# VITA-Group/MM3DGS-SLAM

Hardware: AMD Instinct MI355X
Metric: SLAM frames/sec (track+map), TUM fr1/desk-shaped 640x480 (higher is better)
Workload: dtype f32

## Files before the change

### mm3dgs_slam_amd/csrc/api.hip

```cpp
#include <math.h>
#include <stdarg.h>
#include <stdio.h>
#include <string.h>
#include "mm3dgs_common.h"
#include <algorithm>
#include "fused_api.h"

static thread_local char g_err[512] = "";
static int fail(int code, const char* fmt, ...) {
  va_list ap;
  va_start(ap, fmt);
  vsnprintf(g_err, sizeof(g_err), fmt, ap);
  va_end(ap);
  return code;
}
static int check_launch(const char* what) {
  hipError_t e = hipGetLastError();
  if (e != hipSuccess) return fail(-10, "%s: %s", what, hipGetErrorString(e));
  return 0;
}

#include <mutex>
#include <vector>
struct KernelProfile {
// ... 233 lines not shown
         P > 0 && d.slot_bits >= DIRECT_SLOT_BITS_MIN && T <= max_tiles && T <= MAX_LDS_TILES && d.bin_cap >= 32 && d.rec_cap >= 1024 && d.trec_cap >= 256 &&
         N_capacity >= 4 * (size_t)P;
  return d;
}

static bool slam_tile_table(int flags) { return (flags & MM3DGS_FWD_STATE_CLEAN) && !env_flag("MM3DGS_NO_TILE_ORDER", 0); }
static void slam_refresh_tile_order(const Mm3dgsCamera* cam, void* image_state, int flags, void* stream) {
  if (!cam || !image_state || !slam_tile_table(flags) || cam->image_height <= 0 || cam->image_width <= 0) return;
  if (flags & MM3DGS_FWD_KEEP_TILE_ORDER) return;
  const CamDev cd = cam_dev(cam);
  launch_tile_order(cd.gx * cd.gy, cd.H, cd.W, image_view(image_state, cd.H, cd.W), (hipStream_t)stream);
}

static int slam_forward_impl(const Mm3dgsCamera* cam, int P, const Mm3dgsSlamInputs* in, float* out_color, int32_t* radii,
                             void* geom_state, void* image_state, void* binning_state, size_t N_capacity, int flags, void* stream,
                             const TrackLoss* tl, float* track_dsub = nullptr, bool projected = false, bool pose_chain = false) {
  int rc = check_slam(cam, P, in);
  if (rc) return rc;
  if (!out_color || !geom_state || !image_state || !binning_state || (P > 0 && !radii)) return fail(-1, "NULL buffer");
  hipStream_t s = (hipStream_t)stream;
  CamDev cd = cam_dev(cam);
  GeomView g = geom_view(geom_state, P > 0 ? P : 1);
  ImageView iv = image_view(image_state, cd.H, cd.W);
  BinView b = bin_view(binning_state, N_capacity);
  if (!(flags & MM3DGS_FWD_STATE_CLEAN))
    if (hipMemsetAsync(image_state, 0, iv.zero_bytes, s) != hipSuccess) return fail(-10, "memset failed");
  cd.sort_single = (flags & MM3DGS_FWD_SHORT_LISTS) ? 1 : 0;
  cd.bg_extras = 1;
  cd.state_clean = (flags & MM3DGS_FWD_STATE_CLEAN) ? 1 : 0;
  cd.tile_table = slam_tile_table(flags) ? 1 : 0;
  cd.fused_scan = ((flags & MM3DGS_FWD_STATE_CLEAN) && P > 0 && cd.gx * cd.gy <= MAX_FUSED_SCAN_TILES && !env_flag("MM3DGS_NO_FUSED_SCAN", 0)) ? 1 : 0;
  const bool fused_sort = slam_fused_sort(flags);
  if (tl && !fused_sort) return fail(-1, "internal: folded tracking loss needs the fused sort path");
  const DirectBins db = slam_direct_bins(flags, cd, P, N_capacity);
  cd.trec_cap = db.on ? db.trec_cap : 0u;
  if (db.on) {
    if (!projected) { ProfScope ps(MM3DGS_PROF_PREPROCESS_FWD, s); launch_slam_project_bin(cd, P, slam_in(in), radii, g, iv, b, db.bin_cap, db.rec_cap, db.slot_bits, s, pose_chain); }
    { ProfScope ps(track_dsub ? MM3DGS_PROF_TRACK_FWD_BWD : MM3DGS_PROF_COMPOSITE_FWD, s);
      if (track_dsub) launch_sort_composite_fwd_bwd_track(cd, g, iv, b, N_capacity, out_color, 1, s, *tl, db.nblocks, track_dsub, db.bin_cap, db.slot_bits, pose_chain);
      else launch_sort_composite_fwd6(cd, g, iv, b, N_capacity, out_color, 1, s, tl, db.nblocks, db.bin_cap, db.slot_bits); }
    return check_launch("slam_forward");
  }
  { ProfScope ps(MM3DGS_PROF_PREPROCESS_FWD, s); launch_slam_preprocess_fwd(cd, P, slam_in(in), radii, g, iv, s, nullptr, false, pose_chain); }
  if (!cd.fused_scan) { ProfScope ps(MM3DGS_PROF_SCAN, s); launch_scan_tiles(cd.gx * cd.gy, P, g, iv, s, (flags & MM3DGS_FWD_STATE_CLEAN) ? 1 : 0); }
  { ProfScope ps(MM3DGS_PROF_BIN_SORT, s); launch_scatter_sort(cd, P, g, iv, b, N_capacity, nullptr, s, fused_sort); }
  { ProfScope ps((fused_sort && track_dsub) ? MM3DGS_PROF_TRACK_FWD_BWD : MM3DGS_PROF_COMPOSITE_FWD, s);
    if (fused_sort && track_dsub) launch_sort_composite_fwd_bwd_track(cd, g, iv, b, N_capacity, out_color, (cd.fused_scan || cd.state_clean) ? 1 : 0, s, *tl, 0, track_dsub, 0, DIRECT_SLOT_BITS_MAX, pose_chain);
    else if (fused_sort) launch_sort_composite_fwd6(cd, g, iv, b, N_capacity, out_color, (cd.fused_scan || cd.state_clean) ? 1 : 0, s, tl);
    else launch_composite_fwd(cd, 6, g, iv, b, N_capacity, out_color, s); }
  return check_launch("slam_forward");
}

int mm3dgs_slam_visibility(const Mm3dgsCamera* cam, int P, const Mm3dgsSlamInputs* in, int32_t* radii, uint32_t* seen_count, void* geom_state,
                           void* stream) {
  int rc = check_slam(cam, P, in);
  if (rc) return rc;
  if (!geom_state || (P > 0 && !radii)) return fail(-1, "NULL buffer");
  CamDev cd = cam_dev(cam);
  GeomView g = geom_view(geom_state, P > 0 ? P : 1);
  ImageView iv = {};
  launch_slam_preprocess_fwd(cd, P, slam_in(in), radii, g, iv, (hipStream_t)stream, seen_count, true);
  return check_launch("slam_visibility");
// ... 156 lines not shown
    tl.gt = gt_color; tl.ref = ref; tl.out = out_color; tl.sums = (const double*)w;
    tl.partial = (double*)(w + 256 + align_up((size_t)9 * loss_cfg->H * loss_cfg->W * 4, 256));
    tl.loss4 = loss4;
    tl.defer_scale = loss_cfg->w_pearson == 0.f ? 1 : 0;
    if (loss_cfg->H != cam->image_height || loss_cfg->W != cam->image_width) return fail(-1, "loss and camera image sizes differ");
  }
  const bool fuse_track = fold && tl.defer_scale && !env_flag("MM3DGS_NO_FUSED_TRACK", 0) && backward_scratch;
  float* track_dsub = nullptr;
  if (fuse_track) {
    track_dsub = bwd_view(backward_scratch, P, N_capacity).dsub;
  }
  const bool pose_chain = !in->world_means && !sh && backward_scratch && !env_flag("MM3DGS_NO_POSE_CHAIN", 0) &&
                          bwd_bytes_impl(P, N_capacity) >= (size_t)tiles_x(cam->image_width) * tiles_y(cam->image_height) * 32 * sizeof(float);
  if (n_iter > 0) slam_refresh_tile_order(cam, image_state, fwd_flags, stream);
  for (int it = 0; it < n_iter; it++) {
    int rc = slam_forward_impl(cam, P, in, out_color, radii, geom_state, image_state, binning_state, N_capacity, fwd_flags, stream, fold ? &tl : nullptr, track_dsub, false, pose_chain);
    if (rc) return rc;
    if (fold) {
      if (!tl.defer_scale) {
        ProfScope ps(MM3DGS_PROF_LOSS, (hipStream_t)stream);
        launch_loss_finish(tl.cfg, (double*)loss_work, tl.partial, (hipStream_t)stream);
      }
    } else {
      rc = mm3dgs_loss(loss_cfg, out_color, gt_color, ref, loss_work, dL_dout, loss4, stream);
      if (rc) return rc;
    }
    rc = slam_backward_impl(cam, P, in, radii, geom_state, image_state, binning_state, N_capacity, dL_dout, backward_scratch, &none,
                            nullptr, pose_adam, nullptr, fwd_flags, stream, fold ? &tl : nullptr, loss4, 6, fuse_track, nullptr, nullptr, pose_chain);
    if (rc) return rc;
  }
  return 0;
// ... 229 lines not shown
```

### mm3dgs_slam_amd/csrc/composite.hip

```cpp
#include <type_traits>
#include "mm3dgs_common.h"
#include "sort_tile.h"
#include "fused_api.h"
#include "loss_pixel.h"
#include "loss_tile.h"

#define STG_ROW 17
#define STG_N (4 * STG_ROW)

#include "composite_common.h"

template <int C>
__device__ __forceinline__ void composite_fwd_body(int tile, const CamDev& cam, const GeomView& g, const ImageView& iv, const BinView& b,
                                                   uint32_t N_cap, float* __restrict__ out, float4 (*stg)[4][3][STG_N],
                                                   const uint32_t* counts_lds, const TrackLoss* tl = nullptr,
                                                   double (*red)[12] = nullptr, const SortShared* span = nullptr) {
  const int tid = threadIdx.x, lane = tid & 63, wv = tid >> 6;
  const int row = lane >> 4, q = lane & 15;
  const int slane = row * STG_ROW + q;
  const int px = (tile % cam.gx) * TILE + (wv & 1) * 8 + (row & 1) * 4 + (q & 3);
  const int py = (tile / cam.gx) * TILE + (wv >> 1) * 8 + (row >> 1) * 4 + (q >> 2);
  const bool inside = px < cam.W && py < cam.H;
  const float pxf = (float)px, pyf = (float)py;
  uint32_t start, len;
  if (span) { start = span->start; len = span->len; }
  else tile_span(iv, tile, N_cap, start, len);
  const int L = 4 * wv + row;
  const uint32_t count = len ? min(counts_lds ? counts_lds[L] : iv.subcount[NLIST * tile + L], len) : 0u;
  uint32_t maxcount = count;
  maxcount = max(maxcount, (uint32_t)__builtin_amdgcn_readlane((int)count, 16));
  maxcount = max(maxcount, (uint32_t)__builtin_amdgcn_readlane((int)count, 32));
// ... 62 lines not shown
        splat_fwd(A1, B1, C1, j1);
      }
    }
    if (__ballot(!done && base + CH < count) == 0ull) break;
    stg[cur ^ 1][wv][0][slane] = rec_n.A;
    stg[cur ^ 1][wv][1][slane] = rec_n.B;
    if (C > 2) stg[cur ^ 1][wv][2][slane] = rec_n.C;
    id_nxt = id_nn;
  }
  wave_prio_reset();
  if (cam.stats && lane == 0) atomicAdd(&iv.hdr->fwd_wave_iters, n_iter);
  float fin[C];
#pragma unroll
  for (int ch = 0; ch < C; ch++) fin[ch] = acc[ch] + ((ch < 3 || cam.bg_extras) ? Tr * cam.bg[ch % 3] : 0.f);
  const size_t pix = (size_t)py * cam.W + px, HW = (size_t)cam.H * cam.W;
  if (inside) {
    iv.final_T[pix] = Tr;
    iv.n_contrib[pix] = last_contributor;
#pragma unroll
    for (int ch = 0; ch < C; ch++) out[ch * HW + pix] = fin[ch];
  }
  if constexpr (C == 6) {
    if (tl) {
      double ls[12];
#pragma unroll
      for (int k = 0; k < 12; k++) ls[k] = 0.0;
      if (inside) {
        const float rgb[3] = {fin[0], fin[1], fin[2]};
        const float g3[3] = {tl->gt[pix], tl->gt[HW + pix], tl->gt[2 * HW + pix]};
        loss_px_sums(tl->cfg, rgb, fin[4], fin[3], g3, tl->cfg.w_pearson != 0.f ? tl->ref[pix] : 0.f, ls);
      }
      block_sums<12>(ls, red, pearson_double_cols(tl->cfg));
      if (threadIdx.x == 0) {
        double* rowp = tl->partial + (size_t)tile * 12;
#pragma unroll
        for (int k = 0; k < 12; k++) rowp[k] = ls[k];
      }
    }
  }
}

template <int C>
__global__ void __launch_bounds__(256)
composite_fwd_kernel(CamDev cam, GeomView g, ImageView iv, BinView b, uint32_t N_cap, float* __restrict__ out) {
  __shared__ float4 stg[2][4][3][STG_N];
// ... 92 lines not shown
  static constexpr int OFF_CZ = OFF_B + STG_N * 16;
  static constexpr int OFF_TP = OFF_CZ + STG_N * 8;
  static constexpr int OFF_T5 = OFF_TP + 4 * TP_STRIDE * 8;
  static constexpr int OFF_T = OFF_TP + 8 * TP_STRIDE * 8;
  static constexpr int SLICE = OFF_T + (MODE == 1 ? 64 * 16 : 64 * 4);
};
template <int MODE>
using BwdLds = Bwd2Lds<(MODE == 0 ? 1 : MODE)>;
template <int C, int MODE>
constexpr size_t BWD_WAVE_SLICE = bwd_is_two_phase(MODE, C) ? (size_t)BwdLds<MODE>::SLICE : sizeof(float4) * 3 * STG_N;
template <int C, int MODE>
constexpr size_t BWD_LDS_BYTES = bwd_is_two_phase(MODE, C) ? 4 * (size_t)BwdLds<MODE>::SLICE : (size_t)BWD_STG_BYTES;
template <int C, int MODE, bool POSE = false>
__device__ __forceinline__ void composite_bwd_body(int tile, const CamDev& cam, const GeomView& g, const ImageView& iv, const BinView& b,
                                                   uint32_t N_cap, const float* __restrict__ dL_dout, float* __restrict__ dsub, int has_tl,
                                                   const TrackLoss& tl, int dl_planes, unsigned char* smem_raw, const SortShared* span = nullptr) {
  static_assert(!POSE || MODE == 2, "the pose chain lives in the tracking mode's loop");
  const int tid = threadIdx.x, lane = tid & 63, wv = tid >> 6;
  const int row = lane >> 4, q = lane & 15;
  const int slane = row * STG_ROW + q;
  const int px = (tile % cam.gx) * TILE + (wv & 1) * 8 + (row & 1) * 4 + (q & 3);
  const int py = (tile / cam.gx) * TILE + (wv >> 1) * 8 + (row >> 1) * 4 + (q >> 2);
  const bool inside = px < cam.W && py < cam.H;
  const float pxf = (float)px, pyf = (float)py;
  uint32_t start, len;
  if (span) { start = span->start; len = span->len; }
  else tile_span(iv, tile, N_cap, start, len);
  const int L = 4 * wv + row;
  const uint32_t count = len ? min(span ? span->run[L] : iv.subcount[NLIST * tile + L], len) : 0u;
  const uint2* __restrict__ list = b.sublist + (size_t)NLIST * start + (size_t)L * len;

  constexpr int NV = MODE == 0 ? 6 + C : (MODE == 1 ? 10 : 7);
  static_assert(MODE == 0 || C == 6, "SLAM modes composite the 6-channel bundle");
  constexpr int RECF = MODE == 0 ? GENERIC_RECF(C) : (MODE == 1 ? REC_MAP_F : REC_TRACK_F);
  float4 (*stg)[4][3][STG_N] = (float4 (*)[4][3][STG_N])smem_raw;
  constexpr uint32_t CH = 16;

  const size_t pix = (size_t)py * cam.W + px, HW = (size_t)cam.H * cam.W;
  const float T_final = inside ? iv.final_T[pix] : 0.f;
  const uint32_t last_contributor = inside ? iv.n_contrib[pix] : 0u;
  uint32_t todo = last_contributor;
  todo = max(todo, (uint32_t)__builtin_amdgcn_update_dpp(0, (int)todo, QP_XOR1, 0xf, 0xf, true));
  todo = max(todo, (uint32_t)__builtin_amdgcn_update_dpp(0, (int)todo, QP_XOR2, 0xf, 0xf, true));
  todo = max(todo, (uint32_t)__builtin_amdgcn_update_dpp(0, (int)todo, ROW_ROR4, 0xf, 0xf, true));
  todo = max(todo, (uint32_t)__builtin_amdgcn_update_dpp(0, (int)todo, ROW_ROR8, 0xf, 0xf, true));
  todo = min(todo, count);
  const uint32_t maxtodo = max(max((uint32_t)__builtin_amdgcn_readlane((int)todo, 0), (uint32_t)__builtin_amdgcn_readlane((int)todo, 16)),
                               max((uint32_t)__builtin_amdgcn_readlane((int)todo, 32), (uint32_t)__builtin_amdgcn_readlane((int)todo, 48)));
  float dL[C];
  float bg_dot = 0.f;
  bool dl_done = false;
  if constexpr (MODE == 2) {
    if (has_tl) {
#pragma unroll
      for (int ch = 0; ch < C; ch++) dL[ch] = 0.f;
      if (inside) {
        const float sil = tl.out[4 * HW + pix];
        const bool smask = sil > tl.cfg.sil_thr;
        const float l1s = tl.defer_scale ? tl.cfg.w_l1 / 3.f : loss_l1_scale(tl.cfg, tl.sums);
#pragma unroll
        for (int ch = 0; ch < 3; ch++) dL[ch] = loss_px_l1_grad(tl.cfg, tl.out[ch * HW + pix], tl.gt[ch * HW + pix], smask, l1s);
        if (tl.cfg.w_pearson != 0.f) dL[3] = loss_px_pearson_grad(tl.cfg, sil, tl.out[3 * HW + pix], tl.ref[pix], tl.sums);
      }
      if (!tl.defer_scale && tile == 0 && threadIdx.x == 0 && tl.loss4) loss_scalars(tl.cfg, tl.sums, HW, tl.loss4);
      dl_done = true;
    }
  }
  if constexpr (MODE == 1) {
    if (has_tl) {
      LossGradSmem& lsm = *(LossGradSmem*)smem_raw;
      float* exch = (float*)(smem_raw + sizeof(LossGradSmem));
      float g4[4];
      bool in_raster;
      if (PROBE(cam, 10)) { g4[0] = g4[1] = g4[2] = g4[3] = 1e-3f; in_raster = true; }
      else loss_grad_tile(tl.cfg, tl.out, tl.gt, tl.ref, tl.dmaps, tl.sums, tile, cam.gx, lsm, g4, in_raster);
#pragma unroll
      for (int ch = 0; ch < 4; ch++) exch[ch * 256 + tid] = g4[ch];
// ... 492 lines not shown
  constexpr size_t LOSS_BYTES = MODE == 1 ? sizeof(LossGradSmem) + 4 * 256 * sizeof(float) : 0;
  constexpr size_t MIN_BYTES = MODE == 0 ? 32768 : 0;
  constexpr size_t STG_BYTES = BWD_LDS_BYTES<C, MODE>;
  constexpr size_t NEED = STG_BYTES > LOSS_BYTES ? STG_BYTES : LOSS_BYTES;
  __shared__ __align__(16) unsigned char smem_raw[NEED > MIN_BYTES ? NEED : MIN_BYTES];
  const int T = cam.gx * cam.gy;
  const int tile = slam_tile(cam, iv, blockIdx.x, T);
  if (tile >= T) return;
  if (MODE == 1 && blockIdx.x == 0 && threadIdx.x == 0) iv.hdr->overflow_seen = iv.hdr->overflow;
  composite_bwd_body<C, MODE, POSE>(tile, cam, g, iv, b, N_cap, dL_dout, dsub, has_tl, tl, dl_planes, smem_raw);
}

template <bool POSE>
__global__ void __launch_bounds__(256) __attribute__((amdgpu_waves_per_eu(5, 5)))
sort_composite_fwd_bwd_track_kernel(CamDev cam, GeomView g, ImageView iv, BinView b, uint32_t N_cap, float* __restrict__ out, int clean,
                                    TrackLoss tl, int direct_blocks, float* __restrict__ dsub, uint32_t direct_cap, int slot_bits) {
  constexpr size_t TRACK_BWD_BYTES = BWD_LDS_BYTES<6, 2>;
  __shared__ __align__(16) unsigned char smem[TRACK_BWD_BYTES];
  __shared__ SortShared sh;
  __shared__ double red[4][12];
  static_assert(TRACK_BWD_BYTES >= sizeof(float4) * 2 * 4 * 3 * STG_N, "LDS union too small for the forward staging buffers");
  static_assert(TRACK_BWD_BYTES >= 3 * RANK_SORT_MAX * sizeof(unsigned long long) + sizeof(SortEmit), "LDS union too small for the sort's keys, runs, payloads and the emission's counters");
  const int T = cam.gx * cam.gy;
  const int tile = slam_tile(cam, iv, blockIdx.x, T);
  if (tile >= T) return;
  sort_tile_body<2048, true>(tile, cam.gx, 0, g, iv, b, N_cap, clean, (unsigned long long*)smem, sh, 0, direct_blocks, direct_cap, slot_bits);
  __syncthreads();
  composite_fwd_body<6>(tile, cam, g, iv, b, N_cap, out, (float4 (*)[4][3][STG_N])smem, sh.run, &tl, red, &sh);
  __syncthreads();
  composite_bwd_body<6, 2, POSE>(tile, cam, g, iv, b, N_cap, nullptr, dsub, 1, tl, 6, smem, &sh);
}

template <int C>
static void launch_fwd_c(const CamDev& cam, GeomView g, ImageView iv, BinView b, uint32_t ncap, float* out, hipStream_t s) {
  int T = cam.gx * cam.gy;
  int grid = ((T + 7) / 8) * 8;
  static const int pad = env_flag("MM3DGS_FWD_LDS_PAD", 0);
  hipLaunchKernelGGL((composite_fwd_kernel<C>), dim3(grid), dim3(256), (size_t)pad, s, cam, g, iv, b, ncap, out);
}
template <int C>
static void launch_bwd_c(const CamDev& cam, GeomView g, ImageView iv, BinView b, uint32_t ncap, const float* dL, float* dsub,
                         hipStream_t s) {
  int T = cam.gx * cam.gy;
  int grid = ((T + 7) / 8) * 8;
  TrackLoss none = {};
// ... 13 lines not shown
    hipLaunchKernelGGL((composite_bwd_kernel<6, 2>), dim3(grid), dim3(256), slam_lds_pad(), s, cam, g, iv, b, ncap, dL, dsub, tl ? 1 : 0, tl ? *tl : none, dl_planes);
  else
    hipLaunchKernelGGL((composite_bwd_kernel<6, 1>), dim3(grid), dim3(256), slam_lds_pad(), s, cam, g, iv, b, ncap, dL, dsub, tl ? 1 : 0, tl ? *tl : none, dl_planes);
}

void launch_sort_composite_fwd6(const CamDev& cam, GeomView g, ImageView iv, BinView b, size_t N_cap, float* out, int clean, hipStream_t s,
                                const TrackLoss* tl, int direct_blocks, uint32_t direct_cap, int slot_bits) {
  uint32_t ncap = (uint32_t)(N_cap > 0xffffffffull ? 0xffffffffull : N_cap);
  int T = cam.gx * cam.gy;
  int grid = slam_grid(cam, T);
  TrackLoss none = {};
  hipLaunchKernelGGL((sort_composite_fwd_kernel<6>), dim3(grid), dim3(256), slam_lds_pad(), s, cam, g, iv, b, ncap, out, clean, tl ? 1 : 0, tl ? *tl : none, direct_blocks, direct_cap, slot_bits);
}

void launch_sort_composite_fwd_bwd_track(const CamDev& cam, GeomView g, ImageView iv, BinView b, size_t N_cap, float* out, int clean,
                                         hipStream_t s, const TrackLoss& tl, int direct_blocks, float* dsub, uint32_t direct_cap, int slot_bits, bool pose_chain) {
  uint32_t ncap = (uint32_t)(N_cap > 0xffffffffull ? 0xffffffffull : N_cap);
  int T = cam.gx * cam.gy;
  int grid = slam_grid(cam, T);
  if (pose_chain)
    hipLaunchKernelGGL(sort_composite_fwd_bwd_track_kernel<true>, dim3(grid), dim3(256), slam_lds_pad(), s, cam, g, iv, b, ncap, out, clean, tl, direct_blocks, dsub, direct_cap, slot_bits);
  else
    hipLaunchKernelGGL(sort_composite_fwd_bwd_track_kernel<false>, dim3(grid), dim3(256), slam_lds_pad(), s, cam, g, iv, b, ncap, out, clean, tl, direct_blocks, dsub, direct_cap, slot_bits);
}

void launch_composite_fwd(const CamDev& cam, int C, GeomView g, ImageView iv, BinView b, size_t N_cap, float* out,
                          hipStream_t s) {
  uint32_t ncap = (uint32_t)(N_cap > 0xffffffffull ? 0xffffffffull : N_cap);
  switch (C) {
    case 1: launch_fwd_c<1>(cam, g, iv, b, ncap, out, s); break;
    case 2: launch_fwd_c<2>(cam, g, iv, b, ncap, out, s); break;
    case 3: launch_fwd_c<3>(cam, g, iv, b, ncap, out, s); break;
    case 4: launch_fwd_c<4>(cam, g, iv, b, ncap, out, s); break;
    case 5: launch_fwd_c<5>(cam, g, iv, b, ncap, out, s); break;
    default: launch_fwd_c<6>(cam, g, iv, b, ncap, out, s); break;
  }
}
void launch_composite_bwd(const CamDev& cam, int C, GeomView g, ImageView iv, BinView b, size_t N_cap, const float* dL,
// ... 12 lines not shown
```

### mm3dgs_slam_amd/csrc/fused.hip

```cpp
#pragma clang fp contract(on)
#include "mm3dgs_math.h"
#include "fused_api.h"
#include "composite_common.h"
#include "tile_mask.h"

#define FB 256
#define SLAM_BWD_FB 256
#define SH_C0F 0.28209479177387814f

struct PoseDev { float R[3][3]; float t[3]; float qn[4]; float inv_norm; };

__device__ __forceinline__ PoseDev load_pose(const float* __restrict__ pose) {
  PoseDev p;
  float w = pose[0], x = pose[1], y = pose[2], z = pose[3];
  float n = sqrtf(w * w + x * x + y * y + z * z);
  p.inv_norm = 1.f / n;
  p.qn[0] = w * p.inv_norm; p.qn[1] = x * p.inv_norm; p.qn[2] = y * p.inv_norm; p.qn[3] = z * p.inv_norm;
  quat_to_R(p.qn, p.R);
  p.t[0] = pose[4]; p.t[1] = pose[5]; p.t[2] = pose[6];
  return p;
}

__device__ __forceinline__ void slam_cov3d_vals(const float q[4], const float ls[3], bool isotropic, float mod, float S3[3][3],
                                                float R[3][3], float sm[3], float qn[4], float& qinv) {
// ... 69 lines not shown
  o[3] = make_float4(Kq[2][0], Kq[2][1], Kq[2][2], x[0]);
  o[4] = make_float4(x[1], x[2], 0.f, 0.f);
}

template <int SHDIR>
__device__ __forceinline__ void sh_dir_vec(const PoseDev& ps, const float x[3], const float p[3], float v[3]) {
  static_assert(SHDIR >= 0 && SHDIR <= 2, "sh_dir is 0, 1 or 2");
#pragma unroll
  for (int j = 0; j < 3; j++) {
    if constexpr (SHDIR == 0) v[j] = p[j];
    else if constexpr (SHDIR == 1) v[j] = x[j];
    else v[j] = x[j] + ps.R[0][j] * ps.t[0] + ps.R[1][j] * ps.t[1] + ps.R[2][j] * ps.t[2];
  }
}

template <bool SH = false, int SHDIR = 0>
__device__ __forceinline__ Projected slam_project_vals(const CamDev& cam, bool live, int idx, const float* __restrict__ pose, bool isotropic,
                                                       const RawGaussian& rg, int32_t* __restrict__ radii, const GeomView& g, bool world = false,
                                                       bool want_poserec = false, const float* __restrict__ rest = nullptr, int sh_deg = 0) {
  const float* PV = cam.proj;
  const float Vi[16] = {1.f, 0.f, 0.f, 0.f, 0.f, 1.f, 0.f, 0.f, 0.f, 0.f, 1.f, 0.f, 0.f, 0.f, 0.f, 1.f};
  const PoseDev ps = load_pose(pose);
  float p[3] = {0.f, 0.f, 0.f};
  const float* q_raw = rg.q; const float* ls_raw = rg.ls; const float* fd_raw = rg.fd;
  const float op_raw = rg.op;
  if (live) {
#pragma unroll
    for (int i = 0; i < 3; i++) p[i] = ps.R[i][0] * rg.x[0] + ps.R[i][1] * rg.x[1] + ps.R[i][2] * rg.x[2] + ps.t[i];
  }
  Projected o;
  o.r0 = 0; o.r1 = 0; o.rad = 0; o.z = 0.f; o.cl = 0;
// ... 32 lines not shown
        float c0 = SH_C0F * fd[0] + 0.5f, c1 = SH_C0F * fd[1] + 0.5f, c2 = SH_C0F * fd[2] + 0.5f;
        if constexpr (SH) {
          float v[3];
          sh_dir_vec<SHDIR>(ps, rg.x, p, v);
          const float inv = 1.f / sqrtf(v[0] * v[0] + v[1] * v[1] + v[2] * v[2]);
          float bb[16];
          sh_basis(sh_deg, v[0] * inv, v[1] * inv, v[2] * inv, bb);
          const int nb = (sh_deg + 1) * (sh_deg + 1);
          c0 = bb[0] * fd[0]; c1 = bb[0] * fd[1]; c2 = bb[0] * fd[2];
#pragma unroll
          for (int k = 1; k < 16; k++)
            if (k < nb) { c0 += bb[k] * rest[(k - 1) * 3]; c1 += bb[k] * rest[(k - 1) * 3 + 1]; c2 += bb[k] * rest[(k - 1) * 3 + 2]; }
          c0 += 0.5f; c1 += 0.5f; c2 += 0.5f;
        }
        o.cl = (c0 < 0.f ? 1u : 0u) | (c1 < 0.f ? 2u : 0u) | (c2 < 0.f ? 4u : 0u);
        g.clamped[idx] = (uint8_t)o.cl;
        const float z = p[2];
        const float zc = world ? ps.R[0][2] * rg.x[0] + ps.R[1][2] * rg.x[1] + ps.R[2][2] * rg.x[2] : p[2];
        const float op = 1.f / (1.f + expf(-op_raw));
        float4* sp = (float4*)(g.splat + (size_t)idx * SPLAT_F);
        o.sA = make_float4(px, py, e.c * dinv, -e.b * dinv); o.sB = make_float4(e.a * dinv, op, fmaxf(c0, 0.f), fmaxf(c1, 0.f));
        sp[0] = o.sA;
        sp[1] = o.sB;
        o.br = block_rect(o.sA, o.sB, o.r0, o.r1);
        sp[2] = make_float4(fmaxf(c2, 0.f), zc, 1.f, zc * zc);
        g.depth[idx] = z;
        o.z = z;
        if (want_poserec && !world)
          pose_chain_record(cam, PV, p, rg.x, e, S3, e.c * dinv, -e.b * dinv, e.a * dinv, h.pw, h.hx, h.hy, g.poserec + (size_t)idx * POSEREC_F);
      }
    }
  }
  if (live) {
    radii[idx] = o.rad;
    g.rect[(size_t)idx * 2] = o.r0;
    g.rect[(size_t)idx * 2 + 1] = o.r1;
  }
  return o;
}

template <bool SH = false, int SHDIR = 0>
__device__ __forceinline__ Projected slam_project_one(const CamDev& cam, int P, int idx, const SlamIn& in, int32_t* __restrict__ radii,
                                                      const GeomView& g, bool want_poserec = false) {
  const bool live = idx < P;
  RawGaussian rg = {{0.f, 0.f, 0.f}, {1.f, 0.f, 0.f, 0.f}, {0.f, 0.f, 0.f}, {0.f, 0.f, 0.f}, 0.f};
  if (live) {
#pragma unroll
    for (int k = 0; k < 3; k++) rg.x[k] = in.xyz[(size_t)idx * 3 + k];
#pragma unroll
    for (int k = 0; k < 4; k++) rg.q[k] = in.rotation[(size_t)idx * 4 + k];
#pragma unroll
    for (int k = 0; k < 3; k++) { rg.ls[k] = in.scaling[(size_t)idx * 3 + k]; rg.fd[k] = in.f_dc[(size_t)idx * 3 + k]; }
    rg.op = in.opacity[idx];
  }
  return slam_project_vals<SH, SHDIR>(cam, live, idx, in.pose, in.isotropic != 0, rg, radii, g, in.world != 0, want_poserec,
                               SH ? in.f_rest + (size_t)(live ? idx : 0) * (size_t)in.n_rest * 3 : nullptr, in.sh_deg);
}

template <bool SH, int SHDIR = 0>
__global__ void __launch_bounds__(FB)
slam_preprocess_fwd_kernel(CamDev cam, int P, SlamIn in, int32_t* __restrict__ radii, GeomView g, ImageView iv, int lds_tiles,
                           int vis_only, uint32_t* __restrict__ seen, int want_poserec) {
  extern __shared__ uint32_t hist[];
  const int T = cam.gx * cam.gy;
  for (int t = threadIdx.x; t < lds_tiles; t += FB) hist[t] = 0;
  if (lds_tiles) __syncthreads();
  const int idx = blockIdx.x * FB + threadIdx.x;
  const bool live = idx < P;
  const Projected pr = slam_project_one<SH, SHDIR>(cam, P, idx, in, radii, g, want_poserec != 0);
  const uint32_t r0 = pr.r0, r1 = pr.r1;
// ... 56 lines not shown
};
__device__ __forceinline__ uint32_t emit_pair(const PairCtx& c, int k, int ttx, int tty, uint32_t* hist, int gx, uint32_t cap, const BinView& b,
                                              bool have_mask = false, uint32_t mask_in = 0u) {
  const int t = tty * gx + ttx;
  const uint32_t slot = atomicAdd(&hist[t], 1u);
  uint32_t mask = 0;
  if (slot < cap) {
    mask = have_mask ? mask_in : tile_block_mask_in_rect(c.mc, ttx, tty, c.br);
    const size_t at = (size_t)t * cap + slot;
    b.keys[at] = ((unsigned long long)c.khi << 32) | (unsigned long long)(c.idbits | slot);
    b.payload[at] = (unsigned long long)mask | ((unsigned long long)(c.trec0 == 0xffffffffu ? 0xffffffffu : c.trec0 + (uint32_t)k) << 32);
  }
  return mask;
}

__device__ __forceinline__ void slam_bin_pairs(const CamDev& cam, int P, int idx, const Projected& pr, const GeomView& g, const ImageView& iv,
                                               const BinView& b, uint32_t cap, uint32_t rec_cap, int slot_bits, uint32_t* hist) {
  const int T = cam.gx * cam.gy;
  const int tid = threadIdx.x, lane = tid & 63, wvi = tid >> 6;
  const bool live = idx < P;
  PairCtx c;
  c.mc = mask_consts(pr.sA, pr.sB);
  c.br = pr.br;
  c.minx = pr.r0 & 0xffff; c.miny = pr.r0 >> 16;
  c.w = (int)(pr.r1 & 0xffff) - c.minx;
  c.area = c.w * ((int)(pr.r1 >> 16) - c.miny);
  c.khi = __float_as_uint(pr.z);
  c.idbits = (uint32_t)idx << slot_bits;
  {
    __shared__ uint32_t wtot2[FB / 64];
    const uint32_t x2 = wave_scan_incl((uint32_t)c.area);
    if (lane == 63) wtot2[wvi] = x2;
    __syncthreads();
    uint32_t pre2 = 0;
    for (int q = 0; q < wvi; q++) pre2 += wtot2[q];
    const uint32_t plocal = pre2 + x2 - (uint32_t)c.area;
    if (live) g.tileoff[idx] = plocal;
    c.trec0 = plocal + (uint32_t)c.area <= cam.trec_cap ? (uint32_t)blockIdx.x * cam.trec_cap + plocal : 0xffffffffu;
    if (tid == FB - 1) {
      g.block_tiles[blockIdx.x] = pre2 + x2;
      if (pre2 + x2 > cam.trec_cap) iv.hdr->overflow = 1u;
    }
  }
  constexpr int OWN = 4;
  unsigned long long big = __ballot(c.area > 32);
  unsigned long long m64 = 0ull;
  uint32_t empty4 = 0u;
  const bool droppable = c.area > 0 && c.area <= 32;
  if (droppable) {
    int ttx = c.minx, tty = c.miny;
    const int kmax = PROBE(cam, 7) ? min(c.area, OWN) : c.area;
    for (int k = 0; k < kmax; k++) {
      bool count = true;
      if (k < OWN) {
        const uint32_t mk = tile_block_mask_in_rect(c.mc, ttx, tty, c.br);
        m64 |= (unsigned long long)mk << (16 * k);
        count = mk != 0u;
        empty4 |= count ? 0u : (1u << k);
      }
      if (count) atomicAdd(&hist[tty * cam.gx + ttx], 1u);
      if (++ttx == c.minx + c.w) { ttx = c.minx; tty++; }
    }
  }
  if (live) g.clamped[idx] = (uint8_t)(pr.cl | (empty4 << 4));
  if (PROBE(cam, 8)) big = 0ull;
  for (unsigned long long bb = big; bb; bb &= bb - 1) {
    const int src = __ffsll((long long)bb) - 1;
    const int sminx = __builtin_amdgcn_readlane(c.minx, src), sminy = __builtin_amdgcn_readlane(c.miny, src);
    const int sw = __builtin_amdgcn_readlane(c.w, src), sarea = __builtin_amdgcn_readlane(c.area, src);
    for (int k = lane; k < sarea; k += 64) atomicAdd(&hist[(sminy + k / sw) * cam.gx + sminx + k % sw], 1u);
  }
  __syncthreads();
  for (int t = tid; t < T; t += FB) {
    const uint32_t n = hist[t];
    if (n) hist[t] = atomicAdd(&iv.cursor[t], n);
  }
  __syncthreads();
  {
    int ttx = c.minx, tty = c.miny;
// ... 22 lines not shown
      const PairCtx oc = s_ctx[wvi][o];
      const int k = OWN + (int)(i - excl);
      emit_pair(oc, k, oc.minx + k % oc.w, oc.miny + k / oc.w, hist, cam.gx, cap, b);
    }
  }
}

__device__ __forceinline__ int slam_bin_prologue(const CamDev& cam, const ImageView& iv, uint32_t cap, uint32_t* hist) {
  const int T = cam.gx * cam.gy;
  const int tid = threadIdx.x;
  for (int t = tid; t < T; t += FB) hist[t] = 0;
  if (blockIdx.x == 0 && tid == 0) iv.hdr->bin_cap = cap;
  return blockIdx.x * FB + tid;
}

template <bool SH, int SHDIR = 0>
__global__ void __launch_bounds__(FB)
slam_project_bin_kernel(CamDev cam, int P, SlamIn in, int32_t* __restrict__ radii, GeomView g, ImageView iv, BinView b, uint32_t cap,
                        uint32_t rec_cap, int slot_bits, int want_poserec) {
  extern __shared__ uint32_t hist[];
  const int idx = slam_bin_prologue(cam, iv, cap, hist);
  const Projected pr = slam_project_one<SH, SHDIR>(cam, P, idx, in, radii, g, want_poserec != 0);
  slam_bin_pairs(cam, P, idx, pr, g, iv, b, cap, rec_cap, slot_bits, hist);
}

void launch_slam_project_bin(const CamDev& cam, int P, const SlamIn& in, int32_t* radii, GeomView g, ImageView iv, BinView b, uint32_t bin_cap,
                             uint32_t rec_cap, int slot_bits, hipStream_t s, bool want_poserec) {
  if (P <= 0) return;
  const int T = cam.gx * cam.gy;
  hipLaunchKernelGGL(SLAM_PICK_SH(slam_project_bin_kernel, in), dim3((P + FB - 1) / FB), dim3(FB), (size_t)T * 4, s, cam, P, in, radii, g, iv, b, bin_cap,
                     rec_cap, slot_bits, want_poserec && in.sh_deg <= 0 ? 1 : 0);
}

template <bool TRACK>
__device__ __forceinline__ void gather_tile_records(int area, uint32_t first, const float* __restrict__ dtile, float4& acc0, float4& acc1, float4& acc2,
                                                    uint32_t skip4) {
  constexpr int RECF = TRACK ? REC_TRACK_F : REC_MAP_F;
  const int lane = threadIdx.x & 63;
  const bool big = area > 16;
  const int n_own = big ? 0 : area;
  for (int k0 = 0; __ballot(k0 < n_own) != 0ull; k0 += 4) {
    float4 a[4], b4[4], c4[4];
    bool on[4];
#pragma unroll
// ... 670 lines not shown
```

### mm3dgs_slam_amd/csrc/fused_api.h

```cpp
#pragma once
#include "mm3dgs_common.h"

struct SlamIn {
  const float* pose; const float* xyz; const float* f_dc; const float* opacity; const float* scaling; const float* rotation;
  int isotropic;
  int world;
  const float* f_rest; int sh_deg; int n_rest;
  int sh_dir;
};
struct SlamGrads {
  float* d_xyz; float* d_f_dc; float* d_opacity; float* d_scaling; float* d_rotation;
  float* max_radii2D; float* grad_accum; float* denom;
  float* d_f_rest;
};
struct MapAdam { float* p[5]; float* m[5]; float* v[5]; float step_size[5]; float omb1, beta2, omb2, eps, bc2s; int on; const uint8_t* opt_mask;
                 float* rp; float* rm; float* rv; float rest_step_size; };
struct PoseAdam { float* pose; float* m; float* v; int* step; double lr_q, lr_t, beta1, beta2; float eps; const float* prior; float prior_w_t, prior_w_q; float* best; };
struct AdamGroup { float* p; const float* g; float* m; float* v; unsigned long long n; float step_size; };
struct AdamArgs { AdamGroup grp[8]; int ngroups; float omb1, beta2, omb2, eps, bc2s; };
struct LossCfg {
  int H, W;
  float w_l1, w_ssim, w_pearson;
  int l1_mask, pearson_mask, pearson_invert;
  float sil_thr;
// ... 18 lines not shown
void launch_loss_finish(const LossCfg& cfg, double* sums, const double* partial, hipStream_t s, float* loss4 = nullptr);

void launch_slam_preprocess_fwd(const CamDev& cam, int P, const SlamIn& in, int32_t* radii, GeomView g, ImageView iv, hipStream_t s,
                                uint32_t* seen_only = nullptr, bool visibility_only = false, bool want_poserec = false);
void launch_slam_pose_finish(const float* rows, int nrows, const float* pose_in, float* dpose, const PoseAdam& ad, hipStream_t s,
                             const PoseLossScale* pls, float* loss4, const uint32_t* ovf);
void launch_slam_preprocess_bwd(const CamDev& cam, int P, const SlamIn& in, const int32_t* radii, GeomView g, BinView b, size_t N_cap,
                                BwdView bw, const SlamGrads& out, float* dpose, const PoseAdam& ad, const MapAdam& ma, hipStream_t s,
                                const PoseLossScale* pls = nullptr, float* loss4 = nullptr, bool direct = false, const uint32_t* overflow_flag = nullptr);
void launch_composite_bwd_slam(const CamDev& cam, bool tracking, GeomView g, ImageView iv, BinView b, size_t N_cap, const float* dL,
                               float* dsub, hipStream_t s, const TrackLoss* tl = nullptr, int dl_planes = 6, bool pose_chain = false);
void launch_sort_composite_fwd6(const CamDev& cam, GeomView g, ImageView iv, BinView b, size_t N_cap, float* out, int clean, hipStream_t s,
                                const TrackLoss* tl = nullptr, int direct_blocks = 0, uint32_t direct_cap = 0, int slot_bits = DIRECT_SLOT_BITS_MAX);
void launch_sort_composite_fwd_bwd_track(const CamDev& cam, GeomView g, ImageView iv, BinView b, size_t N_cap, float* out, int clean,
                                         hipStream_t s, const TrackLoss& tl, int direct_blocks, float* dsub, uint32_t direct_cap = 0, int slot_bits = DIRECT_SLOT_BITS_MAX,
                                         bool pose_chain = false);
void launch_slam_bwd_project(const CamDev& cam, int P, const SlamIn& in, int32_t* radii, GeomView g, ImageView iv, BinView b, size_t N_cap,
                             BwdView bw, const SlamGrads& out, const MapAdam& ma, const float* next_pose, uint32_t bin_cap, uint32_t rec_cap,
                             int slot_bits, hipStream_t s);
void launch_slam_project_bin(const CamDev& cam, int P, const SlamIn& in, int32_t* radii, GeomView g, ImageView iv, BinView b, uint32_t bin_cap,
                             uint32_t rec_cap, int slot_bits, hipStream_t s, bool want_poserec = false);
void launch_slam_adam_project(const CamDev& cam, int P, const SlamIn& in, int32_t* radii, GeomView g, ImageView iv, BinView b, const SlamGrads& gr,
                              const MapAdam& ma, const float* next_pose, uint32_t bin_cap, uint32_t rec_cap, int slot_bits, hipStream_t s);
void launch_fused_adam(const AdamArgs& a, hipStream_t s);
void launch_loss(const LossCfg& cfg, const float* out, const float* gt, const float* ref, float* dmaps, double* sums, double* partial,
                 float* dL, float* loss, hipStream_t s);
void launch_loss_after_forward_rows(const LossCfg& cfg, const float* out, const float* gt, const float* ref, float* dmaps, double* sums,
                                    double* partial, float* dL, hipStream_t s);

struct CompactTable { const float* src[32]; float* dst[32]; int width[32]; int n_arrays; };
struct SeedOut { float* xyz; float* f_dc; float* f_rest; float* opacity; float* scaling; float* rotation; float* rgb; int n_rest; };
void launch_prune_mask(int P, const float* opacity, const float* scaling, const float* max_radii2D, float min_opacity, float max_scale,
                       float max_screen_size, int use_screen, uint8_t* keep, uint32_t* n_pruned, hipStream_t s);
void launch_compact_plan(int n, const uint8_t* keep, uint32_t* block_pre, uint32_t* n_keep, hipStream_t s);
void launch_compact_rows(int n, const uint8_t* keep, const uint32_t* block_pre, const CompactTable& t, hipStream_t s);
struct DensifyTable {
// ... 16 lines not shown
```

Before: 31.86.

## Skip per-Gaussian and per-pixel state stores on non-final tracking iterations

Result: no change. 32.09 (median of 6 runs) (+0.7%).

```diff
diff --git a/mm3dgs_slam_amd/csrc/api.hip b/mm3dgs_slam_amd/csrc/api.hip
--- a/mm3dgs_slam_amd/csrc/api.hip
+++ b/mm3dgs_slam_amd/csrc/api.hip
@@ -271,10 +271,11 @@
 
 static int slam_forward_impl(const Mm3dgsCamera* cam, int P, const Mm3dgsSlamInputs* in, float* out_color, int32_t* radii,
                              void* geom_state, void* image_state, void* binning_state, size_t N_capacity, int flags, void* stream,
-                             const TrackLoss* tl, float* track_dsub = nullptr, bool projected = false, bool pose_chain = false) {
+                             const TrackLoss* tl, float* track_dsub = nullptr, bool projected = false, bool pose_chain = false, bool lean = false) {
   int rc = check_slam(cam, P, in);
   if (rc) return rc;
   if (!out_color || !geom_state || !image_state || !binning_state || (P > 0 && !radii)) return fail(-1, "NULL buffer");
+  if (lean && !(track_dsub && pose_chain)) return fail(-1, "internal: a lean iteration is a fused pose-chain tracking iteration");
   hipStream_t s = (hipStream_t)stream;
   CamDev cd = cam_dev(cam);
   GeomView g = geom_view(geom_state, P > 0 ? P : 1);
@@ -292,9 +293,9 @@
   const DirectBins db = slam_direct_bins(flags, cd, P, N_capacity);
   cd.trec_cap = db.on ? db.trec_cap : 0u;
   if (db.on) {
-    if (!projected) { ProfScope ps(MM3DGS_PROF_PREPROCESS_FWD, s); launch_slam_project_bin(cd, P, slam_in(in), radii, g, iv, b, db.bin_cap, db.rec_cap, db.slot_bits, s, pose_chain); }
+    if (!projected) { ProfScope ps(MM3DGS_PROF_PREPROCESS_FWD, s); launch_slam_project_bin(cd, P, slam_in(in), radii, g, iv, b, db.bin_cap, db.rec_cap, db.slot_bits, s, pose_chain, lean); }
     { ProfScope ps(track_dsub ? MM3DGS_PROF_TRACK_FWD_BWD : MM3DGS_PROF_COMPOSITE_FWD, s);
-      if (track_dsub) launch_sort_composite_fwd_bwd_track(cd, g, iv, b, N_capacity, out_color, 1, s, *tl, db.nblocks, track_dsub, db.bin_cap, db.slot_bits, pose_chain);
+      if (track_dsub) launch_sort_composite_fwd_bwd_track(cd, g, iv, b, N_capacity, out_color, 1, s, *tl, db.nblocks, track_dsub, db.bin_cap, db.slot_bits, pose_chain, !lean);
       else launch_sort_composite_fwd6(cd, g, iv, b, N_capacity, out_color, 1, s, tl, db.nblocks, db.bin_cap, db.slot_bits); }
     return check_launch("slam_forward");
   }
@@ -302,7 +303,7 @@
   if (!cd.fused_scan) { ProfScope ps(MM3DGS_PROF_SCAN, s); launch_scan_tiles(cd.gx * cd.gy, P, g, iv, s, (flags & MM3DGS_FWD_STATE_CLEAN) ? 1 : 0); }
   { ProfScope ps(MM3DGS_PROF_BIN_SORT, s); launch_scatter_sort(cd, P, g, iv, b, N_capacity, nullptr, s, fused_sort); }
   { ProfScope ps((fused_sort && track_dsub) ? MM3DGS_PROF_TRACK_FWD_BWD : MM3DGS_PROF_COMPOSITE_FWD, s);
-    if (fused_sort && track_dsub) launch_sort_composite_fwd_bwd_track(cd, g, iv, b, N_capacity, out_color, (cd.fused_scan || cd.state_clean) ? 1 : 0, s, *tl, 0, track_dsub, 0, DIRECT_SLOT_BITS_MAX, pose_chain);
+    if (fused_sort && track_dsub) launch_sort_composite_fwd_bwd_track(cd, g, iv, b, N_capacity, out_color, (cd.fused_scan || cd.state_clean) ? 1 : 0, s, *tl, 0, track_dsub, 0, DIRECT_SLOT_BITS_MAX, pose_chain, !lean);
     else if (fused_sort) launch_sort_composite_fwd6(cd, g, iv, b, N_capacity, out_color, (cd.fused_scan || cd.state_clean) ? 1 : 0, s, tl);
     else launch_composite_fwd(cd, 6, g, iv, b, N_capacity, out_color, s); }
   return check_launch("slam_forward");
@@ -489,7 +490,8 @@
                           bwd_bytes_impl(P, N_capacity) >= (size_t)tiles_x(cam->image_width) * tiles_y(cam->image_height) * 32 * sizeof(float);
   if (n_iter > 0) slam_refresh_tile_order(cam, image_state, fwd_flags, stream);
   for (int it = 0; it < n_iter; it++) {
-    int rc = slam_forward_impl(cam, P, in, out_color, radii, geom_state, image_state, binning_state, N_capacity, fwd_flags, stream, fold ? &tl : nullptr, track_dsub, false, pose_chain);
+    const bool lean = fuse_track && pose_chain && it + 1 < n_iter;
+    int rc = slam_forward_impl(cam, P, in, out_color, radii, geom_state, image_state, binning_state, N_capacity, fwd_flags, stream, fold ? &tl : nullptr, track_dsub, false, pose_chain, lean);
     if (rc) return rc;
     if (fold) {
       if (!tl.defer_scale) {
diff --git a/mm3dgs_slam_amd/csrc/composite.hip b/mm3dgs_slam_amd/csrc/composite.hip
--- a/mm3dgs_slam_amd/csrc/composite.hip
+++ b/mm3dgs_slam_amd/csrc/composite.hip
@@ -10,11 +10,23 @@
 
 #include "composite_common.h"
 
+struct TrackHandoff { float T_final; uint32_t last_contributor; float dL[4]; };
+
+__device__ __forceinline__ void track_px_grad(const TrackLoss& tl, const float (&rgb)[3], float depth, float sil, const float (&gt)[3], size_t pix,
+                                              float (&dL)[4]) {
+  const bool smask = sil > tl.cfg.sil_thr;
+  const float l1s = tl.defer_scale ? tl.cfg.w_l1 / 3.f : loss_l1_scale(tl.cfg, tl.sums);
+#pragma unroll
+  for (int ch = 0; ch < 3; ch++) dL[ch] = loss_px_l1_grad(tl.cfg, rgb[ch], gt[ch], smask, l1s);
+  dL[3] = tl.cfg.w_pearson != 0.f ? loss_px_pearson_grad(tl.cfg, sil, depth, tl.ref[pix], tl.sums) : 0.f;
+}
+
 template <int C>
 __device__ __forceinline__ void composite_fwd_body(int tile, const CamDev& cam, const GeomView& g, const ImageView& iv, const BinView& b,
                                                    uint32_t N_cap, float* __restrict__ out, float4 (*stg)[4][3][STG_N],
                                                    const uint32_t* counts_lds, const TrackLoss* tl = nullptr,
-                                                   double (*red)[12] = nullptr, const SortShared* span = nullptr) {
+                                                   double (*red)[12] = nullptr, const SortShared* span = nullptr, TrackHandoff* ho = nullptr,
+                                                   bool store_image = true) {
   const int tid = threadIdx.x, lane = tid & 63, wv = tid >> 6;
   const int row = lane >> 4, q = lane & 15;
   const int slane = row * STG_ROW + q;
@@ -107,7 +119,7 @@
 #pragma unroll
   for (int ch = 0; ch < C; ch++) fin[ch] = acc[ch] + ((ch < 3 || cam.bg_extras) ? Tr * cam.bg[ch % 3] : 0.f);
   const size_t pix = (size_t)py * cam.W + px, HW = (size_t)cam.H * cam.W;
-  if (inside) {
+  if (inside && store_image) {
     iv.final_T[pix] = Tr;
     iv.n_contrib[pix] = last_contributor;
 #pragma unroll
@@ -122,6 +134,12 @@
         const float rgb[3] = {fin[0], fin[1], fin[2]};
         const float g3[3] = {tl->gt[pix], tl->gt[HW + pix], tl->gt[2 * HW + pix]};
         loss_px_sums(tl->cfg, rgb, fin[4], fin[3], g3, tl->cfg.w_pearson != 0.f ? tl->ref[pix] : 0.f, ls);
+        if (ho) track_px_grad(*tl, rgb, fin[3], fin[4], g3, pix, ho->dL);
+      }
+      if (ho) {
+        ho->T_final = inside ? Tr : 0.f;
+        ho->last_contributor = inside ? last_contributor : 0u;
+        if (!inside) ho->dL[0] = ho->dL[1] = ho->dL[2] = ho->dL[3] = 0.f;
       }
       block_sums<12>(ls, red, pearson_double_cols(tl->cfg));
       if (threadIdx.x == 0) {
@@ -244,7 +262,8 @@
 template <int C, int MODE, bool POSE = false>
 __device__ __forceinline__ void composite_bwd_body(int tile, const CamDev& cam, const GeomView& g, const ImageView& iv, const BinView& b,
                                                    uint32_t N_cap, const float* __restrict__ dL_dout, float* __restrict__ dsub, int has_tl,
-                                                   const TrackLoss& tl, int dl_planes, unsigned char* smem_raw, const SortShared* span = nullptr) {
+                                                   const TrackLoss& tl, int dl_planes, unsigned char* smem_raw, const SortShared* span = nullptr,
+                                                   const TrackHandoff* hin = nullptr) {
   static_assert(!POSE || MODE == 2, "the pose chain lives in the tracking mode's loop");
   const int tid = threadIdx.x, lane = tid & 63, wv = tid >> 6;
   const int row = lane >> 4, q = lane & 15;
@@ -267,8 +286,8 @@
   constexpr uint32_t CH = 16;
 
   const size_t pix = (size_t)py * cam.W + px, HW = (size_t)cam.H * cam.W;
-  const float T_final = inside ? iv.final_T[pix] : 0.f;
-  const uint32_t last_contributor = inside ? iv.n_contrib[pix] : 0u;
+  const float T_final = hin ? hin->T_final : (inside ? iv.final_T[pix] : 0.f);
+  const uint32_t last_contributor = hin ? hin->last_contributor : (inside ? iv.n_contrib[pix] : 0u);
   uint32_t todo = last_contributor;
   todo = max(todo, (uint32_t)__builtin_amdgcn_update_dpp(0, (int)todo, QP_XOR1, 0xf, 0xf, true));
   todo = max(todo, (uint32_t)__builtin_amdgcn_update_dpp(0, (int)todo, QP_XOR2, 0xf, 0xf, true));
@@ -284,13 +303,16 @@
     if (has_tl) {
 #pragma unroll
       for (int ch = 0; ch < C; ch++) dL[ch] = 0.f;
-      if (inside) {
-        const float sil = tl.out[4 * HW + pix];
-        const bool smask = sil > tl.cfg.sil_thr;
-        const float l1s = tl.defer_scale ? tl.cfg.w_l1 / 3.f : loss_l1_scale(tl.cfg, tl.sums);
-#pragma unroll
-        for (int ch = 0; ch < 3; ch++) dL[ch] = loss_px_l1_grad(tl.cfg, tl.out[ch * HW + pix], tl.gt[ch * HW + pix], smask, l1s);
-        if (tl.cfg.w_pearson != 0.f) dL[3] = loss_px_pearson_grad(tl.cfg, sil, tl.out[3 * HW + pix], tl.ref[pix], tl.sums);
+      if (hin) {
+#pragma unroll
+        for (int ch = 0; ch < 4; ch++) dL[ch] = hin->dL[ch];
+      } else if (inside) {
+        const float rgb[3] = {tl.out[pix], tl.out[HW + pix], tl.out[2 * HW + pix]};
+        const float g3[3] = {tl.gt[pix], tl.gt[HW + pix], tl.gt[2 * HW + pix]};
+        float d4[4];
+        track_px_grad(tl, rgb, tl.cfg.w_pearson != 0.f ? tl.out[3 * HW + pix] : 0.f, tl.out[4 * HW + pix], g3, pix, d4);
+#pragma unroll
+        for (int ch = 0; ch < 4; ch++) dL[ch] = d4[ch];
       }
       if (!tl.defer_scale && tile == 0 && threadIdx.x == 0 && tl.loss4) loss_scalars(tl.cfg, tl.sums, HW, tl.loss4);
       dl_done = true;
@@ -813,7 +835,7 @@
 template <bool POSE>
 __global__ void __launch_bounds__(256) __attribute__((amdgpu_waves_per_eu(5, 5)))
 sort_composite_fwd_bwd_track_kernel(CamDev cam, GeomView g, ImageView iv, BinView b, uint32_t N_cap, float* __restrict__ out, int clean,
-                                    TrackLoss tl, int direct_blocks, float* __restrict__ dsub, uint32_t direct_cap, int slot_bits) {
+                                    TrackLoss tl, int direct_blocks, float* __restrict__ dsub, uint32_t direct_cap, int slot_bits, int store_image) {
   constexpr size_t TRACK_BWD_BYTES = BWD_LDS_BYTES<6, 2>;
   __shared__ __align__(16) unsigned char smem[TRACK_BWD_BYTES];
   __shared__ SortShared sh;
@@ -825,9 +847,10 @@
   if (tile >= T) return;
   sort_tile_body<2048, true>(tile, cam.gx, 0, g, iv, b, N_cap, clean, (unsigned long long*)smem, sh, 0, direct_blocks, direct_cap, slot_bits);
   __syncthreads();
-  composite_fwd_body<6>(tile, cam, g, iv, b, N_cap, out, (float4 (*)[4][3][STG_N])smem, sh.run, &tl, red, &sh);
+  TrackHandoff ho;
+  composite_fwd_body<6>(tile, cam, g, iv, b, N_cap, out, (float4 (*)[4][3][STG_N])smem, sh.run, &tl, red, &sh, &ho, store_image != 0);
   __syncthreads();
-  composite_bwd_body<6, 2, POSE>(tile, cam, g, iv, b, N_cap, nullptr, dsub, 1, tl, 6, smem, &sh);
+  composite_bwd_body<6, 2, POSE>(tile, cam, g, iv, b, N_cap, nullptr, dsub, 1, tl, 6, smem, &sh, &ho);
 }
 
 template <int C>
@@ -871,14 +894,15 @@
 }
 
 void launch_sort_composite_fwd_bwd_track(const CamDev& cam, GeomView g, ImageView iv, BinView b, size_t N_cap, float* out, int clean,
-                                         hipStream_t s, const TrackLoss& tl, int direct_blocks, float* dsub, uint32_t direct_cap, int slot_bits, bool pose_chain) {
+                                         hipStream_t s, const TrackLoss& tl, int direct_blocks, float* dsub, uint32_t direct_cap, int slot_bits, bool pose_chain,
+                                         bool store_image) {
   uint32_t ncap = (uint32_t)(N_cap > 0xffffffffull ? 0xffffffffull : N_cap);
   int T = cam.gx * cam.gy;
   int grid = slam_grid(cam, T);
   if (pose_chain)
-    hipLaunchKernelGGL(sort_composite_fwd_bwd_track_kernel<true>, dim3(grid), dim3(256), slam_lds_pad(), s, cam, g, iv, b, ncap, out, clean, tl, direct_blocks, dsub, direct_cap, slot_bits);
+    hipLaunchKernelGGL(sort_composite_fwd_bwd_track_kernel<true>, dim3(grid), dim3(256), slam_lds_pad(), s, cam, g, iv, b, ncap, out, clean, tl, direct_blocks, dsub, direct_cap, slot_bits, store_image ? 1 : 0);
   else
-    hipLaunchKernelGGL(sort_composite_fwd_bwd_track_kernel<false>, dim3(grid), dim3(256), slam_lds_pad(), s, cam, g, iv, b, ncap, out, clean, tl, direct_blocks, dsub, direct_cap, slot_bits);
+    hipLaunchKernelGGL(sort_composite_fwd_bwd_track_kernel<false>, dim3(grid), dim3(256), slam_lds_pad(), s, cam, g, iv, b, ncap, out, clean, tl, direct_blocks, dsub, direct_cap, slot_bits, store_image ? 1 : 0);
 }
 
 void launch_composite_fwd(const CamDev& cam, int C, GeomView g, ImageView iv, BinView b, size_t N_cap, float* out,
diff --git a/mm3dgs_slam_amd/csrc/fused.hip b/mm3dgs_slam_amd/csrc/fused.hip
--- a/mm3dgs_slam_amd/csrc/fused.hip
+++ b/mm3dgs_slam_amd/csrc/fused.hip
@@ -107,7 +107,7 @@
   }
 }
 
-template <bool SH = false, int SHDIR = 0>
+template <bool SH = false, int SHDIR = 0, bool LEAN = false>
 __device__ __forceinline__ Projected slam_project_vals(const CamDev& cam, bool live, int idx, const float* __restrict__ pose, bool isotropic,
                                                        const RawGaussian& rg, int32_t* __restrict__ radii, const GeomView& g, bool world = false,
                                                        bool want_poserec = false, const float* __restrict__ rest = nullptr, int sh_deg = 0) {
@@ -170,7 +170,7 @@
           c0 += 0.5f; c1 += 0.5f; c2 += 0.5f;
         }
         o.cl = (c0 < 0.f ? 1u : 0u) | (c1 < 0.f ? 2u : 0u) | (c2 < 0.f ? 4u : 0u);
-        g.clamped[idx] = (uint8_t)o.cl;
+        if constexpr (!LEAN) g.clamped[idx] = (uint8_t)o.cl;
         const float z = p[2];
         const float zc = world ? ps.R[0][2] * rg.x[0] + ps.R[1][2] * rg.x[1] + ps.R[2][2] * rg.x[2] : p[2];
         const float op = 1.f / (1.f + expf(-op_raw));
@@ -180,14 +180,14 @@
         sp[1] = o.sB;
         o.br = block_rect(o.sA, o.sB, o.r0, o.r1);
         sp[2] = make_float4(fmaxf(c2, 0.f), zc, 1.f, zc * zc);
-        g.depth[idx] = z;
+        if constexpr (!LEAN) g.depth[idx] = z;
         o.z = z;
         if (want_poserec && !world)
           pose_chain_record(cam, PV, p, rg.x, e, S3, e.c * dinv, -e.b * dinv, e.a * dinv, h.pw, h.hx, h.hy, g.poserec + (size_t)idx * POSEREC_F);
       }
     }
   }
-  if (live) {
+  if (live && !LEAN) {
     radii[idx] = o.rad;
     g.rect[(size_t)idx * 2] = o.r0;
     g.rect[(size_t)idx * 2 + 1] = o.r1;
@@ -195,7 +195,7 @@
   return o;
 }
 
-template <bool SH = false, int SHDIR = 0>
+template <bool SH = false, int SHDIR = 0, bool LEAN = false>
 __device__ __forceinline__ Projected slam_project_one(const CamDev& cam, int P, int idx, const SlamIn& in, int32_t* __restrict__ radii,
                                                       const GeomView& g, bool want_poserec = false) {
   const bool live = idx < P;
@@ -209,7 +209,7 @@
     for (int k = 0; k < 3; k++) { rg.ls[k] = in.scaling[(size_t)idx * 3 + k]; rg.fd[k] = in.f_dc[(size_t)idx * 3 + k]; }
     rg.op = in.opacity[idx];
   }
-  return slam_project_vals<SH, SHDIR>(cam, live, idx, in.pose, in.isotropic != 0, rg, radii, g, in.world != 0, want_poserec,
+  return slam_project_vals<SH, SHDIR, LEAN>(cam, live, idx, in.pose, in.isotropic != 0, rg, radii, g, in.world != 0, want_poserec,
                                SH ? in.f_rest + (size_t)(live ? idx : 0) * (size_t)in.n_rest * 3 : nullptr, in.sh_deg);
 }
 
@@ -296,6 +296,7 @@
   return mask;
 }
 
+template <bool LEAN = false>
 __device__ __forceinline__ void slam_bin_pairs(const CamDev& cam, int P, int idx, const Projected& pr, const GeomView& g, const ImageView& iv,
                                                const BinView& b, uint32_t cap, uint32_t rec_cap, int slot_bits, uint32_t* hist) {
   const int T = cam.gx * cam.gy;
@@ -317,8 +318,8 @@
     uint32_t pre2 = 0;
     for (int q = 0; q < wvi; q++) pre2 += wtot2[q];
     const uint32_t plocal = pre2 + x2 - (uint32_t)c.area;
-    if (live) g.tileoff[idx] = plocal;
-    c.trec0 = plocal + (uint32_t)c.area <= cam.trec_cap ? (uint32_t)blockIdx.x * cam.trec_cap + plocal : 0xffffffffu;
+    if (live && !LEAN) g.tileoff[idx] = plocal;
+    c.trec0 = LEAN ? 0xffffffffu : plocal + (uint32_t)c.area <= cam.trec_cap ? (uint32_t)blockIdx.x * cam.trec_cap + plocal : 0xffffffffu;
     if (tid == FB - 1) {
       g.block_tiles[blockIdx.x] = pre2 + x2;
       if (pre2 + x2 > cam.trec_cap) iv.hdr->overflow = 1u;
@@ -344,7 +345,7 @@
       if (++ttx == c.minx + c.w) { ttx = c.minx; tty++; }
     }
   }
-  if (live) g.clamped[idx] = (uint8_t)(pr.cl | (empty4 << 4));
+  if (live && !LEAN) g.clamped[idx] = (uint8_t)(pr.cl | (empty4 << 4));
   if (PROBE(cam, 8)) big = 0ull;
   for (unsigned long long bb = big; bb; bb &= bb - 1) {
     const int src = __ffsll((long long)bb) - 1;
@@ -397,20 +398,25 @@
   return blockIdx.x * FB + tid;
 }
 
-template <bool SH, int SHDIR = 0>
+template <bool SH, int SHDIR = 0, bool LEAN = false>
 __global__ void __launch_bounds__(FB)
 slam_project_bin_kernel(CamDev cam, int P, SlamIn in, int32_t* __restrict__ radii, GeomView g, ImageView iv, BinView b, uint32_t cap,
                         uint32_t rec_cap, int slot_bits, int want_poserec) {
   extern __shared__ uint32_t hist[];
   const int idx = slam_bin_prologue(cam, iv, cap, hist);
-  const Projected pr = slam_project_one<SH, SHDIR>(cam, P, idx, in, radii, g, want_poserec != 0);
-  slam_bin_pairs(cam, P, idx, pr, g, iv, b, cap, rec_cap, slot_bits, hist);
+  const Projected pr = slam_project_one<SH, SHDIR, LEAN>(cam, P, idx, in, radii, g, want_poserec != 0);
+  slam_bin_pairs<LEAN>(cam, P, idx, pr, g, iv, b, cap, rec_cap, slot_bits, hist);
 }
 
 void launch_slam_project_bin(const CamDev& cam, int P, const SlamIn& in, int32_t* radii, GeomView g, ImageView iv, BinView b, uint32_t bin_cap,
-                             uint32_t rec_cap, int slot_bits, hipStream_t s, bool want_poserec) {
+                             uint32_t rec_cap, int slot_bits, hipStream_t s, bool want_poserec, bool lean) {
   if (P <= 0) return;
   const int T = cam.gx * cam.gy;
+  if (lean && want_poserec && in.sh_deg <= 0) {
+    hipLaunchKernelGGL((slam_project_bin_kernel<false, 0, true>), dim3((P + FB - 1) / FB), dim3(FB), (size_t)T * 4, s, cam, P, in, radii, g, iv, b, bin_cap,
+                       rec_cap, slot_bits, 1);
+    return;
+  }
   hipLaunchKernelGGL(SLAM_PICK_SH(slam_project_bin_kernel, in), dim3((P + FB - 1) / FB), dim3(FB), (size_t)T * 4, s, cam, P, in, radii, g, iv, b, bin_cap,
                      rec_cap, slot_bits, want_poserec && in.sh_deg <= 0 ? 1 : 0);
 }
diff --git a/mm3dgs_slam_amd/csrc/fused_api.h b/mm3dgs_slam_amd/csrc/fused_api.h
--- a/mm3dgs_slam_amd/csrc/fused_api.h
+++ b/mm3dgs_slam_amd/csrc/fused_api.h
@@ -56,12 +56,12 @@
                                 const TrackLoss* tl = nullptr, int direct_blocks = 0, uint32_t direct_cap = 0, int slot_bits = DIRECT_SLOT_BITS_MAX);
 void launch_sort_composite_fwd_bwd_track(const CamDev& cam, GeomView g, ImageView iv, BinView b, size_t N_cap, float* out, int clean,
                                          hipStream_t s, const TrackLoss& tl, int direct_blocks, float* dsub, uint32_t direct_cap = 0, int slot_bits = DIRECT_SLOT_BITS_MAX,
-                                         bool pose_chain = false);
+                                         bool pose_chain = false, bool store_image = true);
 void launch_slam_bwd_project(const CamDev& cam, int P, const SlamIn& in, int32_t* radii, GeomView g, ImageView iv, BinView b, size_t N_cap,
                              BwdView bw, const SlamGrads& out, const MapAdam& ma, const float* next_pose, uint32_t bin_cap, uint32_t rec_cap,
                              int slot_bits, hipStream_t s);
 void launch_slam_project_bin(const CamDev& cam, int P, const SlamIn& in, int32_t* radii, GeomView g, ImageView iv, BinView b, uint32_t bin_cap,
-                             uint32_t rec_cap, int slot_bits, hipStream_t s, bool want_poserec = false);
+                             uint32_t rec_cap, int slot_bits, hipStream_t s, bool want_poserec = false, bool lean = false);
 void launch_slam_adam_project(const CamDev& cam, int P, const SlamIn& in, int32_t* radii, GeomView g, ImageView iv, BinView b, const SlamGrads& gr,
                               const MapAdam& ma, const float* next_pose, uint32_t bin_cap, uint32_t rec_cap, int slot_bits, hipStream_t s);
 void launch_fused_adam(const AdamArgs& a, hipStream_t s);
```
